# rayglover-ibm/sparse-solvers

Measured on AMD Instinct MI355X. Metric: signals recovered/sec (Homotopy l1, m=8192 n=65536 k=64 fp32), higher is better.
Workload: dtype f32; 1 GPU; configs[1]: one signal per solve, A 8192x65536 fp32 = default_rng(1234).standard_normal/sqrt(m) (SURVEY 8d recipe), k=64 positive coefficients, tol 1e-3, max_iter 256; shipped defaults (reference behaviour: tie_guard 0, zero_on_removal 0); m=8192, n=65536, k=64, sweep_variant=5, engine=1

## Files before the change

### sparse-solvers_amd/csrc/resident.hip

```cpp
#include "ss_hip_internal.h"
#include "ss_hip_device.h"
#include "resident.h"

#include <hip/hip_fp16.h>

#include <algorithm>
#include <cmath>
#include <cstdio>
#include <cstdlib>
#include <cstring>

namespace sship {

template <typename T> struct ResVec;
template <> struct ResVec<double> { typedef double v2 __attribute__((ext_vector_type(2))); };
template <> struct ResVec<float>  { typedef float v2 __attribute__((ext_vector_type(2))); };

template <typename T>
struct ResLds {
    T* I;
    T* dvec;
    T* xvec;
    T* u1sg;
    T* u2w;
    int32_t* posof;
    uint32_t* subc;
    uint32_t* pcol;
    uint32_t* psub;
};

template <typename T>
__host__ __device__ inline size_t res_lds_bytes()
{
    typedef ResCfg<T> C;
    return ((size_t)C::PCAP * (C::PCAP + 1) + 6 * (size_t)C::PCAP) * sizeof(T) + ((size_t)2 * C::S + 2 * (size_t)C::PCAP) * 4;
}

template <typename T> __device__ __forceinline__ T res_sqrt(T v);
template <> __device__ __forceinline__ float res_sqrt<float>(float v) { return sqrtf(v); }
template <> __device__ __forceinline__ double res_sqrt<double>(double v) { return sqrt(v); }
template <typename T> __device__ __forceinline__ T res_fma(T a, T b, T c);
template <> __device__ __forceinline__ float res_fma<float>(float a, float b, float c) { return __builtin_fmaf(a, b, c); }
template <> __device__ __forceinline__ double res_fma<double>(double a, double b, double c) { return __builtin_fma(a, b, c); }
template <typename T> __device__ __forceinline__ T res_abs(T v) { return v < T(0) ? -v : v; }

__device__ __forceinline__ uint32_t uni(uint32_t v) { return (uint32_t)__builtin_amdgcn_readfirstlane((int)v); }
__device__ __forceinline__ int32_t uni(int32_t v) { return __builtin_amdgcn_readfirstlane(v); }
__device__ __forceinline__ float uni(float v) { return __uint_as_float(uni(__float_as_uint(v))); }
__device__ __forceinline__ double uni(double v)
{
    const uint32_t lo = uni((uint32_t)__double2loint(v)), hi = uni((uint32_t)__double2hiint(v));
    return __hiloint2double((int)hi, (int)lo);
}


__device__ __forceinline__ void cmov_inplace(float& dst, float src, unsigned long long msk)
{
    asm volatile("v_cndmask_b32_e64 %0, %0, %1, %2" : "+v"(dst) : "v"(src), "s"(msk));
}
__device__ __forceinline__ void cmov_inplace(double& dst, double src, unsigned long long msk)
{
    uint32_t lo = (uint32_t)__double2loint(dst), hi = (uint32_t)__double2hiint(dst);
    const uint32_t slo = (uint32_t)__double2loint(src), shi = (uint32_t)__double2hiint(src);
    asm volatile("v_cndmask_b32_e64 %0, %0, %2, %4\n\tv_cndmask_b32_e64 %1, %1, %3, %4" : "+v"(lo), "+v"(hi) : "v"(slo), "v"(shi), "s"(msk));
    dst = __hiloint2double((int)hi, (int)lo);
}

template <typename T>
__device__ __forceinline__ T group8_sum(T v)
{
    v += dpp_mov<kDppXor1>(v);
    v += dpp_mov<kDppXor2>(v);
    v += dpp_mov<kDppHalfMirror>(v);
    return v;
}

template <typename T>
__device__ __forceinline__ T wave_max_val(T v)
{
    { const T o = dpp_mov<kDppXor1>(v); v = o > v ? o : v; }
    { const T o = dpp_mov<kDppXor2>(v); v = o > v ? o : v; }
    { const T o = dpp_mov<kDppHalfMirror>(v); v = o > v ? o : v; }
    { const T o = dpp_mov<kDppMirror>(v); v = o > v ? o : v; }
    T b = lane_value(v, 0);
#pragma unroll
    for (int r = 1; r < 4; ++r) { const T o = lane_value(v, 16 * r); b = o > b ? o : b; }
    return b;
}

constexpr uint32_t kPickNone = 0xffffu;
template <typename T> struct alignas(16) ResPick { T v; uint32_t who; uint32_t col; };
static_assert(sizeof(ResPick<float>) == 16 && sizeof(ResPick<double>) == 16, "one 16-byte read per wave");

template <typename T, bool OMP, bool STAMPS = false>
__global__ __launch_bounds__(ResCfg<T>::THREADS)
void k_res_solve(const T* __restrict__ Gs_all, uint32_t gpitch, size_t g_slot_stride, const T* __restrict__ c0_all, uint32_t c0_stride,
                 const uint32_t* __restrict__ sub_all, uint32_t n, T tol, uint32_t max_iter, int strict_sign, int tie_guard, int tie_exit,
                 uint32_t kcap, uint32_t* __restrict__ log_hdr, T* __restrict__ log_H, uint32_t* __restrict__ log_pcol, T* __restrict__ log_X, T* __restrict__ log_D,
                 T* __restrict__ x_all, uint32_t x_stride, uint32_t* __restrict__ gam2_all, uint32_t* __restrict__ touched2_all,
                 DevState* __restrict__ st_all, TraceEntry* trace, uint32_t trace_cap, unsigned long long* dbg = nullptr)
{
    unsigned long long tph[6] = { 0, 0, 0, 0, 0, 0 };
    unsigned long long tlast = 0;
#define RES_STAMP(PH) if constexpr (STAMPS) { const unsigned long long now_ = __builtin_readcyclecounter(); tph[PH] += now_ - tlast; tlast = now_; }
    typedef ResCfg<T> C;
    typedef typename ResVec<T>::v2 V2;
    constexpr uint32_t S = C::S, THREADS = C::THREADS, PCAP = C::PCAP, LOGCAP = C::LOGCAP;
    constexpr int CT = C::CT, PT = C::PCAP / 8;
    constexpr uint32_t NW = (THREADS + 63) / 64;
    constexpr uint32_t IP = PCAP + 1u;
    static_assert(THREADS / 8 * CT == S, "eight lanes per column group");
    static_assert(PCAP % 8 == 0 && (CT == 4 || CT == 8), "positions dealt out over the eight lanes of a group");
    extern __shared__ __attribute__((aligned(16))) unsigned char smem[];
    __shared__ T s_max[16];
    __shared__ ResPick<T> s_pick[NW];
    __shared__ T s_f[4];
    ResLds<T> L;
    {
        T* p = reinterpret_cast<T*>(smem);
        L.I = p; p += (size_t)PCAP * IP;
        L.dvec = p; p += PCAP; L.xvec = p; p += PCAP; L.u1sg = p; p += 2 * PCAP; L.u2w = p; p += 2 * PCAP;
        L.posof = reinterpret_cast<int32_t*>(p);
        L.subc = reinterpret_cast<uint32_t*>(L.posof + S);
        L.pcol = L.subc + S;
        L.psub = L.pcol + PCAP;
    }
    const uint32_t slot = blockIdx.x, t = threadIdx.x, lane = t & 63u, wave = t >> 6;
    const uint32_t grp = t >> 3, g = t & 7u;
    const T* Gs = Gs_all + (size_t)slot * g_slot_stride;
    const T* c0 = c0_all + (size_t)slot * c0_stride;
    const uint32_t* sub = sub_all + (size_t)slot * S;
    T* x_out = x_all + (size_t)slot * x_stride;
    uint32_t* gam_out = gam2_all + (size_t)slot * 2 * kcap;
    uint32_t* tch_out = touched2_all + (size_t)slot * 2 * kcap;
    DevState* st = st_all + slot;
    uint32_t* hdr = log_hdr + (size_t)slot * LOGCAP * 8;
    T* LH = log_H != nullptr ? log_H + (size_t)slot * LOGCAP * 2 : nullptr;
    T* LX = log_X + (size_t)slot * LOGCAP * PCAP;
    T* LD = log_D != nullptr ? log_D + (size_t)slot * LOGCAP * PCAP : nullptr;
    if (slot != 0) trace = nullptr;

    const uint32_t jc0 = grp * (uint32_t)CT;
    const bool owner = g < (uint32_t)CT;
    const uint32_t myj = jc0 + (g & (uint32_t)(CT - 1));
    const uint32_t mycol = sub[myj];
    const bool myvalid = owner && mycol < n;
    const T my_c0 = mycol < n ? c0[mycol] : T(0);
    T my_c = my_c0, my_q = T(0);
    int32_t mypos = -1;
    T gr[CT][PT];
#pragma unroll
    for (int c = 0; c < CT; ++c)
#pragma unroll
        for (int e = 0; e < PT; ++e) gr[c][e] = T(0);
    for (uint32_t j = t; j < S; j += THREADS) { L.subc[j] = sub[j]; L.posof[j] = -1; }
    for (uint32_t p = t; p < PCAP; p += THREADS) {
        L.dvec[p] = T(0); L.xvec[p] = T(0); L.pcol[p] = 0xffffffffu; L.psub[p] = 0u;
        L.u1sg[2 * p] = T(0); L.u1sg[2 * p + 1] = T(0); L.u2w[2 * p] = T(0); L.u2w[2 * p + 1] = T(0);
    }
    for (uint32_t e = t; e < PCAP * IP; e += THREADS) L.I[e] = T(0);
    T warm = T(0);
    {
        const size_t gbytes = (size_t)S * gpitch * sizeof(T);
        const unsigned char* gb = reinterpret_cast<const unsigned char*>(Gs);
#pragma unroll 4
        for (size_t off = (size_t)t * 128u; off < gbytes; off += (size_t)THREADS * 128u) warm += *reinterpret_cast<const T*>(gb + off);
    }

    auto publish_pick = [&](T v, T ext, bool tiew) __attribute__((always_inline)) {
        const unsigned long long bal = __builtin_amdgcn_ballot_w64(v == ext);
        const uint32_t src = bal != 0ull ? (uint32_t)__builtin_ctzll(bal) : 0u;
        if (lane == src) {
            ResPick<T> sl;
            sl.v = ext;
            sl.who = (myvalid ? myj : kPickNone) | ((uint32_t)(mypos + 1) << 16) | (tiew ? 0x80000000u : 0u);
            sl.col = mycol;
            s_pick[wave] = sl;
        }
    };
    auto gather_pick = [&](bool want_min, T& v, uint32_t& i, uint32_t& col, int32_t& pos, bool& tie) __attribute__((always_inline)) {
        ResPick<T> sl[NW];
#pragma unroll
        for (uint32_t w = 0; w < NW; ++w) sl[w] = s_pick[w];
        T bv = sl[0].v;
        uint32_t bw = sl[0].who, bc = sl[0].col, ties = sl[0].who;
#pragma unroll
        for (uint32_t w = 1; w < NW; ++w) {
            const bool take = want_min ? sl[w].v < bv : sl[w].v > bv;
            bv = take ? sl[w].v : bv; bw = take ? sl[w].who : bw; bc = take ? sl[w].col : bc;
            ties |= sl[w].who;
        }
        v = uni(bv);
        const uint32_t who = uni((bw & 0x7fffffffu) | (ties & 0x80000000u));
        col = uni(bc);
        i = (who & 0xffffu) == kPickNone ? 0xffffffffu : (who & 0xffffu);
        pos = (int32_t)((who >> 16) & 0x7fffu) - 1;
        tie = (who >> 31) != 0u;
    };
    auto block_min = [&](T m, bool tie, T& v, uint32_t& i, uint32_t& col, int32_t& pos, bool& anytie) __attribute__((always_inline)) {
        publish_pick(m, -wave_max_val<T>(-m), __builtin_amdgcn_ballot_w64(tie) != 0ull);
        lds_barrier();
        gather_pick(true, v, i, col, pos, anytie);
    };
    auto block_argmax = [&](T m, T& v, uint32_t& i, uint32_t& col, int32_t& pos) __attribute__((always_inline)) {
        const T wv = wave_max_val<T>(m);
        lds_barrier();
        publish_pick(m, wv, false);
        lds_barrier();
        bool none;
        gather_pick(false, v, i, col, pos, none);
        lds_barrier();
    };
    auto border_inverse = [&](uint32_t P, T dvv) __attribute__((always_inline)) {
        constexpr uint32_t RW = PCAP / 2u + 1u;
        constexpr uint32_t NG = THREADS / RW;
        const uint32_t Pn = P + 1u;
        const uint32_t pa = t % RW, vg = t / RW;
        const uint32_t a0 = pa, a1 = Pn - 1u - pa;
        if (P != 0xffffffffu && vg < NG && 2u * pa < Pn + 1u - 0u && a0 <= a1) {
            const uint32_t n0 = Pn - a0;
            const uint32_t ntot = a0 == a1 ? n0 : n0 + (Pn - a1);
            const T u0 = a0 < P ? L.u2w[2 * a0] : T(0), u1v = a1 < P ? L.u2w[2 * a1] : T(0);
            constexpr uint32_t BU = sizeof(T) == 8 ? 2u : 3u;
            auto where = [&](uint32_t k, uint32_t& a, uint32_t& b, T& ua) __attribute__((always_inline)) {
                const bool first = k < n0;
                a = first ? a0 : a1;
                b = first ? a0 + k : a1 + (k - n0);
                ua = first ? u0 : u1v;
            };
            auto value = [&](uint32_t a, uint32_t b, T ua, T iv, T ub) __attribute__((always_inline)) -> T {
                const T edge = a == P ? dvv : -dvv * ua;
                const T inner = iv + (dvv * ua) * ub;
                return b == P ? edge : inner;
            };
            uint32_t k = vg;
#pragma nounroll
            for (; k + (BU - 1u) * NG < ntot; k += BU * NG) {
                uint32_t ea[BU], eb[BU];
                T ua[BU], iv[BU], ub[BU];
#pragma unroll
                for (uint32_t u = 0; u < BU; ++u) {
                    where(k + u * NG, ea[u], eb[u], ua[u]);
                    iv[u] = L.I[ea[u] * IP + eb[u]];
                    ub[u] = L.u2w[2 * eb[u]];
                }
#pragma unroll
                for (uint32_t u = 0; u < BU; ++u) {
                    const T val = value(ea[u], eb[u], ua[u], iv[u], ub[u]);
                    L.I[ea[u] * IP + eb[u]] = val;
                    L.I[eb[u] * IP + ea[u]] = val;
                }
            }
#pragma nounroll
            for (; k < ntot; k += NG) {
                uint32_t ea, eb;
                T ua;
                where(k, ea, eb, ua);
                const T val = value(ea, eb, ua, L.I[ea * IP + eb], L.u2w[2 * eb]);
                L.I[ea * IP + eb] = val;
                L.I[eb * IP + ea] = val;
            }
        }
    };

    struct RowVals { T mine; T gv[CT]; };
    auto row_fetch = [&](uint32_t spi, RowVals& rv) __attribute__((always_inline)) {
        const T* row = Gs + (size_t)spi * gpitch;
        rv.mine = row[myj];
        if constexpr (sizeof(T) == 8) {
            const v2d a = *reinterpret_cast<const v2d*>(row + jc0), b = *reinterpret_cast<const v2d*>(row + jc0 + 2);
            rv.gv[0] = a[0]; rv.gv[1] = a[1]; rv.gv[2] = b[0]; rv.gv[3] = b[1];
        } else {
            const v4f a = *reinterpret_cast<const v4f*>(row + jc0), b = *reinterpret_cast<const v4f*>(row + jc0 + 4);
#pragma unroll
            for (int e = 0; e < 4; ++e) { rv.gv[e] = a[e]; rv.gv[4 + e] = b[e]; }
        }
        asm volatile("" ::: "memory");
    };
    auto row_place = [&](uint32_t Pn, const RowVals& rv) __attribute__((always_inline)) {
        const uint32_t e_new = uni(Pn >> 3);
        const unsigned long long msk = __builtin_amdgcn_ballot_w64(g == (Pn & 7u));
#pragma unroll
        for (int c = 0; c < CT; ++c) asm volatile("" :: "v"(rv.gv[c]));
        asm volatile("" :: "v"(rv.mine));
        if constexpr (CT == 8) {
#define RES_CM(I) "v_cndmask_b32_e64 %[d" #I "], %[d" #I "], %[s" #I "], %[m]\n\t"
#pragma unroll
            for (int e = 0; e < PT; ++e) {
                const uint32_t off = uni(e_new ^ (uint32_t)e);
                asm volatile("s_cmp_lg_u32 %[off], 0\n\t"
                             "s_cbranch_scc1 .Lres_place_%=\n\t"
                             RES_CM(0) RES_CM(1) RES_CM(2) RES_CM(3) RES_CM(4) RES_CM(5) RES_CM(6) RES_CM(7)
                             ".Lres_place_%=:"
                             : [d0] "+v"(gr[0][e]), [d1] "+v"(gr[1][e]), [d2] "+v"(gr[2][e]), [d3] "+v"(gr[3][e]), [d4] "+v"(gr[4][e]), [d5] "+v"(gr[5][e]),
                               [d6] "+v"(gr[6][e]), [d7] "+v"(gr[7][e])
                             : [s0] "v"(rv.gv[0]), [s1] "v"(rv.gv[1]), [s2] "v"(rv.gv[2]), [s3] "v"(rv.gv[3]), [s4] "v"(rv.gv[4]), [s5] "v"(rv.gv[5]),
                               [s6] "v"(rv.gv[6]), [s7] "v"(rv.gv[7]), [m] "s"(msk), [off] "s"(off)
                             : "scc");
            }
#undef RES_CM
        } else {
#pragma unroll
            for (int e = 0; e < PT; ++e) {
                if (e_new == (uint32_t)e) {
#pragma unroll
                    for (int c = 0; c < CT; ++c) cmov_inplace(gr[c][e], rv.gv[c], msk);
                }
            }
        }
    };
    auto chain = [&](const T* vec, uint32_t P) __attribute__((always_inline)) -> T {
        T acc[CT];
#pragma unroll
        for (int c = 0; c < CT; ++c) acc[c] = T(0);
#pragma unroll
        for (int e = 0; e < PT; ++e) {
            if ((uint32_t)(8 * e) < P) {
                const T dval = vec[8 * e + (int)g];
#pragma unroll
                for (int c = 0; c < CT; ++c) acc[c] = res_fma<T>(dval, gr[c][e], acc[c]);
            }
        }
        T h4[4];
        if constexpr (CT == 8) {
            const bool up = (g & 4u) != 0u;
#pragma unroll
            for (int i = 0; i < 4; ++i) {
                const T keep = up ? acc[4 + i] : acc[i], send = up ? acc[i] : acc[4 + i];
                h4[i] = keep + dpp_mov<kDppHalfMirror>(send);
            }
        } else {
#pragma unroll
            for (int i = 0; i < 4; ++i) h4[i] = acc[i] + dpp_mov<kDppHalfMirror>(acc[i]);
        }
        const bool b1 = (g & 2u) != 0u, b0 = (g & 1u) != 0u;
        const T k0 = (b1 ? h4[2] : h4[0]) + dpp_mov<kDppXor2>(b1 ? h4[0] : h4[2]);
        const T k1 = (b1 ? h4[3] : h4[1]) + dpp_mov<kDppXor2>(b1 ? h4[1] : h4[3]);
        return (b0 ? k1 : k0) + dpp_mov<kDppXor1>(b0 ? k0 : k1);
    };
    auto inverse_pass = [&](uint32_t P) __attribute__((always_inline)) {
        constexpr int CH = sizeof(T) == 8 ? 6 : PT;
        for (uint32_t a = grp; a < P; a += THREADS / 8u) {
            const T* row = L.I + (size_t)a * IP + g;
            const T* us = L.u1sg + 2u * g;
            T s1 = T(0), s2 = T(0);
#pragma nounroll
            for (int e0 = 0; e0 < PT; e0 += CH) {
                if ((uint32_t)(8 * e0) < P) {
                    T iv[CH];
                    V2 pr[CH];
#pragma unroll
                    for (int e = 0; e < CH; ++e) {
                        if (e0 + e < PT) {
                            iv[e] = row[8 * (e0 + e)];
                            pr[e] = *reinterpret_cast<const V2*>(&us[16 * (e0 + e)]);
                        } else { iv[e] = T(0); pr[e] = V2{ T(0), T(0) }; }
                    }
#pragma unroll
                    for (int e = 0; e < CH; ++e) {
                        s1 = res_fma<T>(iv[e], pr[e][0], s1);
                        s2 = res_fma<T>(iv[e], pr[e][1], s2);
                    }
                }
            }
            s1 = group8_sum<T>(s1); s2 = group8_sum<T>(s2);
            if (g == 0) { L.u2w[2 * a] = s1; L.u2w[2 * a + 1] = s2; }
        }
    };
    auto two_dots = [&](uint32_t P, T& d1, T& d2) __attribute__((always_inline)) {
        T a1 = T(0), a2 = T(0);
#pragma nounroll
        for (uint32_t b = lane; b < P; b += 64u) {
            const V2 pr = *reinterpret_cast<const V2*>(&L.u1sg[2 * b]);
            const T u2b = L.u2w[2 * b];
            a1 = res_fma<T>(pr[0], u2b, a1);
            a2 = res_fma<T>(u2b, pr[1], a2);
        }
        d1 = wave_sum<T>(a1); d2 = wave_sum<T>(a2);
    };
    asm volatile("" : "+s"(trace_cap));
    uint32_t P = 0, status = 0, iter = 0, nlog = 0, reason = 0;
    T c_inf = T(0), lambda_prev = T(0), gamma_prev = T(0), lambda0 = T(0);
    bool tie_any = false;
    lds_barrier();

    uint32_t sp0;
    {
        uint32_t col0;
        int32_t pos0;
        block_argmax(myvalid ? res_abs<T>(my_c) : T(-1), lambda0, sp0, col0, pos0);
    }
    if (sp0 >= S) { status = kStatusSubsetDecline; reason |= kReasonNoCand; }
    else {
        RowVals rv0;
        row_fetch(sp0, rv0);
        row_place(0u, rv0);
        const T g00 = rv0.mine;
        if (owner && myj == sp0) {
            const T nrm = res_sqrt<T>(g00);
            const T inv00 = T(1) / (nrm * nrm);
            const T seed = strict_sign ? my_c : res_abs<T>(my_c);
            const T sg0 = sign_tol<T>(seed, tol);
            L.I[0] = inv00;
            if (OMP) L.xvec[0] = inv00 * my_c; else L.dvec[0] = inv00 * sg0;
            L.pcol[0] = mycol; L.psub[0] = sp0; L.posof[sp0] = 0;
            mypos = 0;
            if (!OMP && trace != nullptr) { trace[0].idx = mycol; trace[0].added = 1; trace[0].gamma = 0.0; trace[0].c_inf = (double)res_abs<T>(my_c); }
        }
        P = 1;
        c_inf = lambda0;
        lambda_prev = lambda0;
        if (!((double)tol >= (sizeof(T) == 8 ? kGramGuard64 : kGramGuard) * (double)lambda0)) { status = kStatusSubsetDecline; reason |= kReasonGuard; }
        lds_barrier();
    }

    if constexpr (OMP) {
        if (status == 0u && !(lambda0 > tol)) { status = kStatusSubsetDecline; reason |= kReasonNoCand; }
        if (status == 0u) {
            if (t == 0) {
                uint32_t* h = hdr;
                h[0] = 0u; h[1] = 1u; h[2] = L.subc[sp0]; h[3] = 1u; h[4] = __float_as_uint((float)lambda0); h[5] = 0u; h[6] = 0xffffffffu; h[7] = 0u;
                if (LH != nullptr) { LH[0] = lambda0; LH[1] = T(0); }
                if (trace != nullptr && 1u < trace_cap) { trace[1].idx = L.subc[sp0]; trace[1].added = 1u; trace[1].gamma = 0.0; trace[1].c_inf = (double)lambda0; }
            }
            if (t < PCAP) LX[t] = T(0);
            nlog = 1;
            iter = 1;
        }
        for (uint32_t round = 2; status == 0u; ++round) {
            my_c = my_c0 - chain(L.xvec, P);
            uint32_t bi, idx;
            int32_t wpos;
            block_argmax(myvalid ? res_abs<T>(my_c) : T(-1), c_inf, bi, idx, wpos);
            const uint32_t spi = bi < S ? bi : 0u;
            RowVals rv;
            row_fetch(spi, rv);
            const bool stop = !(c_inf > tol) || round > max_iter;
            const bool logfull = nlog >= LOGCAP;
            const bool stall_c = bi >= S || wpos >= 0;
            const bool full_c = P >= PCAP || P + 1u > kcap;
            uint32_t verdict = full_c ? kReasonPositions : 0u;
            verdict = stall_c ? (uint32_t)kReasonNoCand : verdict;
            verdict = stop ? 0u : verdict;
            verdict = logfull ? (uint32_t)kReasonLog : verdict;
            const bool ok = !stop && verdict == 0u;
            const bool ends = stop && !logfull;
            status = verdict != 0u ? (uint32_t)kStatusSubsetDecline : ends ? 0xffffffffu : status;
            reason |= verdict;
            iter = ends ? round - 1 : iter;
            row_place(ok ? P : 0xffffffffu, rv);
            const T my_g = rv.mine;
            if (owner && mypos >= 0) { L.u1sg[2 * mypos] = my_g; L.u1sg[2 * mypos + 1] = my_c0; }
            if (ok && owner && myj == spi) { s_f[0] = my_g; s_f[1] = my_c0; L.posof[spi] = (int32_t)P; L.pcol[P] = idx; L.psub[P] = spi; mypos = (int32_t)P; }
            lds_barrier();
            if (!logfull) {
                if (t == 0) {
                    uint32_t* h = hdr + nlog * 8;
                    h[0] = P; h[1] = stop ? 0u : 1u; h[2] = ok ? idx : 0xffffffffu; h[3] = ok ? 1u : 0u; h[4] = __float_as_uint((float)c_inf); h[5] = 0u;
                    h[6] = 0xffffffffu; h[7] = 0u;
                    if (LH != nullptr) { LH[nlog * 2] = c_inf; LH[nlog * 2 + 1] = T(0); }
                    if (ok && trace != nullptr && round < trace_cap) { trace[round].idx = idx; trace[round].added = 1u; trace[round].gamma = 0.0; trace[round].c_inf = (double)c_inf; }
                }
                if (t < PCAP) LX[(size_t)nlog * PCAP + t] = t < P ? L.xvec[t] : T(0);
                ++nlog;
            }
            inverse_pass(P);
            lds_barrier();
            T d1, d2;
            two_dots(P, d1, d2);
            const T dvv = T(1) / (s_f[0] - d1);
            const T beta = dvv * (s_f[1] - d2);
            if (ok && t < P) L.xvec[t] = L.u2w[2 * t + 1] - beta * L.u2w[2 * t];
            if (ok && t == P) L.xvec[P] = beta;
            border_inverse(ok ? P : 0xffffffffu, dvv);
            lds_barrier();
            if (ok) { P += 1u; iter = round; }
        }
        if (status == 0xffffffffu) status = 0u;
    } else {
        if (status == 0u) my_q = chain(L.dvec, P);
        uint32_t pendP = 0xffffffffu;
        T pend_dv = T(0);
        constexpr uint32_t TL0 = THREADS - ((PCAP + 63u) / 64u) * 64u;
        const uint32_t tl = t - TL0;
        for (uint32_t round = 1; status == 0u; ++round) {
            if constexpr (STAMPS) tlast = __builtin_readcyclecounter();
            const bool stop = (round > 1 && !(c_inf > tol)) || round > max_iter;
            const bool logfull = nlog >= LOGCAP;
            const bool in_band = tie_band<T>(c_inf, lambda_prev, gamma_prev, lambda0);
            T m = Lim<T>::max();
            bool tie = false;
            if (myvalid) {
                if (mypos >= 0) {
                    const T tt = -L.xvec[mypos] / L.dvec[mypos];
                    if (tt > T(0) && tt < m) m = tt;
                } else {
                    const T dl = T(1) - my_q, dr = T(1) + my_q;
                    if (dl != T(0)) {
                        T tt = (c_inf - my_c) / dl;
                        if (tie_guard && tt == T(0) && dl > T(0)) tt = Lim<T>::tiny();
                        if (tt == T(0) && in_band) tie = true;
                        if (tt > T(0) && tt < m) m = tt;
                    }
                    if (dr != T(0)) {
                        T tt = (c_inf + my_c) / dr;
                        if (tie_guard && tt == T(0) && dr > T(0)) tt = Lim<T>::tiny();
                        if (tt == T(0) && in_band) tie = true;
                        if (tt > T(0) && tt < m) m = tt;
                    }
                }
            }
            T gmm;
            uint32_t bi, idx;
            int32_t wpos;
            bool anytie;
            block_min(m, tie, gmm, bi, idx, wpos, anytie);
            RES_STAMP(0)
            const uint32_t spi = bi < S ? bi : 0u;
            RowVals rv;
            row_fetch(spi, rv);
            tie_any = tie_any || (!stop && anytie);
            const bool tied_c = tie_any && tie_exit != 0;
            const bool nocand_c = bi >= S || !(gmm < Lim<T>::max());
            const bool full_c = P >= PCAP || P + 1u > kcap;
            uint32_t verdict = full_c ? kReasonPositions : 0u;
            verdict = wpos >= 0 ? (uint32_t)kReasonRemoval : verdict;
            verdict = nocand_c ? (uint32_t)kReasonNoCand : verdict;
            verdict = tied_c ? (uint32_t)kReasonTie : verdict;
            verdict = stop ? 0u : verdict;
            verdict = logfull ? (uint32_t)kReasonLog : verdict;
            const bool ok = !stop && verdict == 0u;
            const bool ends = stop && !logfull;
            const bool tied = verdict == kReasonTie;
            status = ends ? 0xffffffffu : tied ? (uint32_t)kStatusTieRerun : verdict != 0u ? (uint32_t)kStatusSubsetDecline : status;
            reason |= verdict;
            iter = ends || tied ? round - 1 : iter;
            T xv = T(0), dv = T(0);
            if (tl < P) { xv = L.xvec[tl]; dv = L.dvec[tl]; }
            border_inverse(pendP, pend_dv);
            pendP = 0xffffffffu;
            if (ok && tl < P) L.xvec[tl] = xv + gmm * dv;
            if (ok) my_c = res_fma<T>(-gmm, my_q, my_c);
            {
                const T mx = wave_max_val<T>(myvalid ? res_abs<T>(my_c) : T(-1));
                if (lane == 0) s_max[wave] = mx;
            }
            row_place(ok ? P : 0xffffffffu, rv);
            const T my_g = rv.mine;
            if (owner && mypos >= 0) { L.u1sg[2 * mypos] = my_g; L.u1sg[2 * mypos + 1] = sign_tol<T>(my_c, tol); }
            if (ok && owner && myj == spi) {
                s_f[0] = my_g; s_f[1] = sign_tol<T>(my_c, tol);
                L.posof[spi] = (int32_t)P; L.pcol[P] = idx; L.psub[P] = spi; mypos = (int32_t)P;
            }
            lds_barrier();
            RES_STAMP(1)
            if (!logfull) {
                if (tl == 0u) {
                    uint32_t* h = hdr + nlog * 8;
                    h[0] = P; h[1] = stop ? 0u : 1u; h[2] = ok ? idx : 0xffffffffu; h[3] = ok ? 1u : 0u; h[4] = __float_as_uint((float)c_inf);
                    h[5] = ok ? __float_as_uint((float)gmm) : 0u; h[6] = 0xffffffffu; h[7] = in_band ? 1u : 0u;
                    if (LH != nullptr) { LH[nlog * 2] = c_inf; LH[nlog * 2 + 1] = ok ? gmm : T(0); }
                    if (ok && trace != nullptr && round < trace_cap) { trace[round].idx = idx; trace[round].added = 1u; trace[round].gamma = (double)gmm; trace[round].c_inf = (double)c_inf; }
                }
                if (tl < PCAP) {
                    LX[(size_t)nlog * PCAP + tl] = xv;
                    if (LD != nullptr) LD[(size_t)nlog * PCAP + tl] = dv;
                }
                if (stop || tied || ok) ++nlog;
            }
            T c_next = s_max[0];
#pragma unroll
            for (uint32_t w = 1; w < NW; ++w) { const T o = s_max[w]; c_next = o > c_next ? o : c_next; }
            c_next = uni(c_next);
            inverse_pass(P);
            lds_barrier();
            RES_STAMP(2)
            T d1, d2;
            two_dots(P, d1, d2);
            const T dvv = T(1) / (s_f[0] - d1);
            const T beta = dvv * (s_f[1] - d2);
            if (ok && t < P) L.dvec[t] = L.u2w[2 * t + 1] - beta * L.u2w[2 * t];
            if (ok && t == P) L.dvec[P] = beta;
            pendP = ok ? P : 0xffffffffu;
            pend_dv = dvv;
            lds_barrier();
            RES_STAMP(3)
            if (ok) {
                P += 1u;
                lambda_prev = c_inf;
                gamma_prev = gmm;
                c_inf = c_next;
                iter = round;
            }
            my_q = chain(L.dvec, P);
            RES_STAMP(4)
            if constexpr (STAMPS) tph[5] += 1;
        }
        if (status == 0xffffffffu) status = 0u;
    }
    if constexpr (STAMPS) {
        if (dbg != nullptr && slot == 0u && t == 0u)
            for (int q = 0; q < 6; ++q) dbg[q] = tph[q];
    }
#undef RES_STAMP
    lds_barrier();
    if (t < PCAP) log_pcol[(size_t)slot * PCAP + t] = t < P ? L.pcol[t] : 0xffffffffu;
    if (status == 0u || status == kStatusTieRerun) {
        if (t < P) {
            const uint32_t col = L.pcol[t];
            uint32_t rk = 0;
#pragma nounroll
            for (uint32_t b = 0; b < P; ++b) rk += L.pcol[b] < col ? 1u : 0u;
            gam_out[rk] = col;
            tch_out[rk] = col;
            x_out[col] = L.xvec[t];
        }
    }
    if (t == 0) {
        st->done = 1;
        st->status = status;
        st->iter = iter;
        st->K = P;
        st->ntouched = P;
        st->cur = 0;
        st->c_inf = (double)c_inf;
        st->gamma = (double)gamma_prev;
        st->tie_stall = tie_any ? 1u : 0u;
        st->lambda0 = (float)lambda0;
        st->solo_nlog = nlog;
        st->need_sweep = 0;
        st->done_round = iter + 1u;
        st->sub_reason = reason;
    }
    if (warm == T(1.2345e-30)) st->pad4_[0] = 1u;
}

constexpr uint32_t kG64T = 64, kG64Step = 32, kG64Pitch = kG64Step + 1;
typedef double res_v4d __attribute__((ext_vector_type(4)));

__global__ __launch_bounds__(256)
void k_sgram64_part(const double* __restrict__ At, uint32_t ldm, uint32_t n, const uint32_t* __restrict__ sub, uint32_t rows_per,
                    double* __restrict__ part)
{
    constexpr uint32_t S = ResCfg<double>::S;
    __shared__ double sI[kG64T][kG64Pitch];
    __shared__ double sJ[kG64T][kG64Pitch];
    sub += (size_t)blockIdx.z * S;
    part += (size_t)blockIdx.z * gridDim.y * S * S;
    const uint32_t b = blockIdx.x;
    uint32_t tt = (uint32_t)((__fsqrt_rn(8.f * (float)b + 1.f) - 1.f) * 0.5f);
    while (tt * (tt + 1u) / 2u > b) --tt;
    while ((tt + 1u) * (tt + 2u) / 2u <= b) ++tt;
    const uint32_t bj = tt, bi = b - tt * (tt + 1u) / 2u;
    const uint32_t chunk = blockIdx.y;
    const uint32_t tid = threadIdx.x, lane = tid & 63u, w = tid >> 6;
    const uint32_t wi = w >> 1, wj = w & 1u;
    const uint32_t sc = tid >> 2, sq = tid & 3u;
    const uint32_t ci = sub[bi * kG64T + sc], cj = sub[bj * kG64T + sc];
    const bool oki = ci < n, okj = cj < n;
    const double* gi = At + (size_t)(oki ? ci : 0u) * ldm + (size_t)chunk * rows_per + 8u * sq;
    const double* gj = At + (size_t)(okj ? cj : 0u) * ldm + (size_t)chunk * rows_per + 8u * sq;
    const v2d zero2 = { 0.0, 0.0 };
    v2d vi[4], vj[4];
#define SG64_LOAD(R0)                                                                         \
    _Pragma("unroll") for (int p = 0; p < 4; ++p) {                                           \
        vi[p] = oki ? *reinterpret_cast<const v2d*>(gi + (R0) + 2 * p) : zero2;               \
        vj[p] = okj ? *reinterpret_cast<const v2d*>(gj + (R0) + 2 * p) : zero2;               \
    }
    SG64_LOAD(0u)
    res_v4d acc[2][2];
#pragma unroll
    for (int i = 0; i < 2; ++i)
#pragma unroll
        for (int j = 0; j < 2; ++j) acc[i][j] = res_v4d{ 0.0, 0.0, 0.0, 0.0 };
    const uint32_t l15 = lane & 15u, kq = lane >> 4;
    for (uint32_t r0 = 0; r0 < rows_per; r0 += kG64Step) {
        __syncthreads();
#pragma unroll
        for (int p = 0; p < 4; ++p) {
            sI[sc][8u * sq + 2u * (uint32_t)p] = vi[p][0]; sI[sc][8u * sq + 2u * (uint32_t)p + 1u] = vi[p][1];
            sJ[sc][8u * sq + 2u * (uint32_t)p] = vj[p][0]; sJ[sc][8u * sq + 2u * (uint32_t)p + 1u] = vj[p][1];
        }
        __syncthreads();
        if (r0 + kG64Step < rows_per) SG64_LOAD(r0 + kG64Step)
#pragma unroll
        for (uint32_t k4 = 0; k4 < kG64Step; k4 += 4) {
            const double a0 = sI[32u * wi + l15][k4 + kq], a1 = sI[32u * wi + 16u + l15][k4 + kq];
            const double b0 = sJ[32u * wj + l15][k4 + kq], b1 = sJ[32u * wj + 16u + l15][k4 + kq];
            acc[0][0] = __builtin_amdgcn_mfma_f64_16x16x4f64(a0, b0, acc[0][0], 0, 0, 0);
            acc[0][1] = __builtin_amdgcn_mfma_f64_16x16x4f64(a0, b1, acc[0][1], 0, 0, 0);
            acc[1][0] = __builtin_amdgcn_mfma_f64_16x16x4f64(a1, b0, acc[1][0], 0, 0, 0);
            acc[1][1] = __builtin_amdgcn_mfma_f64_16x16x4f64(a1, b1, acc[1][1], 0, 0, 0);
        }
    }
#undef SG64_LOAD
    double* Pp = part + (size_t)chunk * S * S;
#pragma unroll
    for (int i = 0; i < 2; ++i)
#pragma unroll
        for (int j = 0; j < 2; ++j)
#pragma unroll
            for (int e = 0; e < 4; ++e) {
                const uint32_t row = bi * kG64T + 32u * wi + 16u * (uint32_t)i + 4u * (uint32_t)e + kq;
                const uint32_t col = bj * kG64T + 32u * wj + 16u * (uint32_t)j + l15;
                Pp[(size_t)row * S + col] = acc[i][j][e];
                if (bi != bj) Pp[(size_t)col * S + row] = acc[i][j][e];
            }
}

__global__ __launch_bounds__(256)
void k_sgram64_sum(const double* __restrict__ part, uint32_t nsplit, double* __restrict__ gs, const double* __restrict__ At, uint32_t ldm,
                   const double* __restrict__ y, const uint32_t* __restrict__ sub, uint32_t n, double* __restrict__ c0, uint32_t c0_stride)
{
    constexpr uint32_t S = ResCfg<double>::S;
    constexpr uint32_t NB = S * S / 256u;
    {
        const size_t slot = blockIdx.y;
        part += slot * nsplit * S * S; gs += slot * S * S; y += slot * ldm; sub += slot * S; c0 += slot * c0_stride;
    }
    if (blockIdx.x >= NB) {
        __shared__ double sv[16];
        const uint32_t col = sub[blockIdx.x - NB];
        const double* a = At + (size_t)(col < n ? col : 0u) * ldm;
        double acc = 0.0;
        for (uint32_t r0 = 2u * threadIdx.x; r0 < ldm; r0 += 8u * 512u) {
            v2d av[8], yv[8];
#pragma unroll
            for (int q = 0; q < 8; ++q) {
                const uint32_t r = r0 + 512u * (uint32_t)q;
                av[q] = r < ldm ? *reinterpret_cast<const v2d*>(a + r) : v2d{ 0.0, 0.0 };
                yv[q] = r < ldm ? *reinterpret_cast<const v2d*>(y + r) : v2d{ 0.0, 0.0 };
            }
#pragma unroll
            for (int q = 0; q < 8; ++q) { acc = __builtin_fma(av[q][0], yv[q][0], acc); acc = __builtin_fma(av[q][1], yv[q][1], acc); }
        }
        acc = block_sum(acc, sv);
        if (threadIdx.x == 0u && col < n) c0[col] = acc;
        return;
    }
    const uint32_t i = blockIdx.x * 256u + threadIdx.x;
    double s = part[i];
    for (uint32_t c = 1; c < nsplit; ++c) s += part[(size_t)c * S * S + i];
    gs[i] = s;
}

constexpr uint32_t kR64Rhs = 192;
__device__ __forceinline__ float res_state_scale(float lam_eff)
{
    int e = 12;
    if (lam_eff > 0.f && lam_eff < 3.0e38f) e = (int)floorf(log2f(4096.f / lam_eff));
    e = e < -100 ? -100 : (e > 100 ? 100 : e);
    return ldexpf(1.f, e);
}

__global__ __launch_bounds__(256)
void k_res_residuals64(const double* __restrict__ At, uint32_t ldm, uint32_t n, const double* __restrict__ y, const uint32_t* __restrict__ hdr,
                       const double* __restrict__ LH, const uint32_t* __restrict__ pcol, const double* __restrict__ LX, double tol,
                       const float* __restrict__ meta, __half* __restrict__ r16, float* __restrict__ rn2p, float* __restrict__ tab,
                       uint32_t* __restrict__ headroom, DevState* __restrict__ st, int first16, int omp, const float* __restrict__ slotmeta,
                       uint32_t* __restrict__ fl, int scan)
{
    constexpr uint32_t kFlCap = kScrFlCap;
    constexpr uint32_t PCAP = ResCfg<double>::PCAP;
    constexpr uint32_t LOGCAP = ResCfg<double>::LOGCAP;
    constexpr uint32_t XP = kR64Rhs + 8u;
    {
        const size_t slot = blockIdx.y;
        y += slot * ldm; hdr += slot * LOGCAP * 8; LH += slot * LOGCAP * 2; pcol += slot * PCAP; LX += slot * LOGCAP * PCAP;
        r16 += slot * kR64Rhs * ldm; rn2p += slot * (ldm / 64u) * kR64Rhs; tab += slot * kR64Rhs * 4u; st += slot;
        if (slotmeta != nullptr) slotmeta += slot * 4u;
    }
    __shared__ __attribute__((aligned(16))) double sAc[16][64];
    __shared__ __attribute__((aligned(16))) double sXt[16][XP];
    __shared__ float sS[kR64Rhs];
    if (st->status != 0u && !scan) return;
    const uint32_t tid = threadIdx.x, r0 = blockIdx.x * 64u;
    const uint32_t nlog = st->solo_nlog;
    float ratio0 = 0.f;
    if (fl != nullptr && blockIdx.x == 0u && blockIdx.y == 0u && tid == 0u) {
        fl[0] = 0u; fl[kFlCap + 1u] = 0u; fl[kFlCap + 4u] = 0u; fl[kFlCap + 12u] = 0u; fl[kFlCap + 13u] = 0u;
        if (!scan) fl[kFlCap + 14u] = 0u;
    }
    if (first16 && !scan && blockIdx.x == 0u && tid == 0u && nlog >= 1u) {
        const float lam0 = (float)LH[0] * 0.9999999f;
        const float yn = sqrtf(slotmeta != nullptr ? slotmeta[0] : meta[5]) * 1.001f;
        float eps0 = slotmeta != nullptr ? 0.0019726562f * yn * meta[4] + 6.103515625e-05f * sqrtf((float)ldm) * yn * meta[1]
                                         : meta[8] * yn * meta[4] + meta[9] * sqrtf((float)ldm) * yn;
        if (slotmeta != nullptr) eps0 += 6.103515625e-05f * sqrtf((float)ldm) * meta[4] * slotmeta[2];
        const float bound0 = lam0 * 0.875f - 1e-12f * lam0;
        const float v0 = (slotmeta != nullptr ? slotmeta[1] : meta[6]) + eps0;
        if (!(v0 <= bound0)) {
            if (fl != nullptr && bound0 > 0.f) { fl[kFlCap + 1u] = 1u; fl[kFlCap + 2u] = __float_as_uint(bound0); fl[kFlCap + 3u] = __float_as_uint(eps0); }
            else { __hip_atomic_store(&st->need_sweep, 1u, __ATOMIC_RELAXED, __HIP_MEMORY_SCOPE_AGENT); atomicOr(&st->sub_reason, kReasonFirstState); }
        }
        ratio0 = bound0 > 0.f && v0 == v0 ? v0 / bound0 : 3.0e38f;
    }
    if (nlog < 2u) {
        if (blockIdx.x == 0u && tid == 0u && blockIdx.y == 0u) *headroom = __float_as_uint(ratio0);
        return;
    }
    const uint32_t nst = nlog - 1u;
    if (nst > kR64Rhs) {
        if (blockIdx.x == 0u && tid == 0u && !scan) { __hip_atomic_store(&st->need_sweep, 1u, __ATOMIC_RELAXED, __HIP_MEMORY_SCOPE_AGENT); atomicOr(&st->sub_reason, kReasonLog); }
        return;
    }
    const uint32_t Pfin = hdr[(size_t)(nlog - 1u) * 8u];
    if (tid < kR64Rhs) {
        float sc = 1.f;
        if (tid < nst) {
            const double lam = LH[(size_t)(tid + 1u) * 2u];
            const bool final_state = !(hdr[(size_t)(tid + 1u) * 8u + 1u] & 1u);
            sc = res_state_scale((float)(final_state ? fmax(lam, tol) : lam));
        }
        sS[tid] = sc;
    }
    const uint32_t rg = tid & 15u, sgp = tid >> 4;
    double acc[3][4][4];
    {
        const v2d y0 = *reinterpret_cast<const v2d*>(y + r0 + 4u * rg), y1 = *reinterpret_cast<const v2d*>(y + r0 + 4u * rg + 2u);
#pragma unroll
        for (int rd = 0; rd < 3; ++rd)
#pragma unroll
            for (int si = 0; si < 4; ++si) { acc[rd][si][0] = y0[0]; acc[rd][si][1] = y0[1]; acc[rd][si][2] = y1[0]; acc[rd][si][3] = y1[1]; }
    }
    for (uint32_t u0 = 0; u0 < Pfin; u0 += 16u) {
        __syncthreads();
        {
            const uint32_t p = tid >> 4, q4 = tid & 15u;
            const uint32_t u = u0 + p;
            const uint32_t col = u < Pfin ? pcol[u] : 0xffffffffu;
            v2d a0 = { 0.0, 0.0 }, a1 = { 0.0, 0.0 };
            if (col < n) {
                a0 = *reinterpret_cast<const v2d*>(At + (size_t)col * ldm + r0 + 4u * q4);
                a1 = *reinterpret_cast<const v2d*>(At + (size_t)col * ldm + r0 + 4u * q4 + 2u);
            }
            *reinterpret_cast<v2d*>(&sAc[p][4u * q4]) = a0;
            *reinterpret_cast<v2d*>(&sAc[p][4u * q4 + 2u]) = a1;
            for (uint32_t e = tid; e < 16u * XP; e += 256u) {
                const uint32_t k = e / 16u, pp = e - k * 16u;
                sXt[pp][k] = (u0 + pp < Pfin && k < nst) ? LX[(size_t)(k + 1u) * PCAP + u0 + pp] : 0.0;
            }
        }
        __syncthreads();
#pragma unroll
        for (int rd = 0; rd < 3; ++rd) {
            const uint32_t s0 = 64u * (uint32_t)rd + 4u * sgp;
            if (s0 < nst) {
#pragma unroll 4
                for (uint32_t p = 0; p < 16u; ++p) {
                    const v2d a0 = *reinterpret_cast<const v2d*>(&sAc[p][4u * rg]), a1 = *reinterpret_cast<const v2d*>(&sAc[p][4u * rg + 2u]);
                    const v2d x0 = *reinterpret_cast<const v2d*>(&sXt[p][s0]), x1 = *reinterpret_cast<const v2d*>(&sXt[p][s0 + 2u]);
                    const double av[4] = { a0[0], a0[1], a1[0], a1[1] }, xv[4] = { x0[0], x0[1], x1[0], x1[1] };
#pragma unroll
                    for (int si = 0; si < 4; ++si)
#pragma unroll
                        for (int ri = 0; ri < 4; ++ri) acc[rd][si][ri] = __builtin_fma(-xv[si], av[ri], acc[rd][si][ri]);
                }
            }
        }
    }
    const double units = (double)meta[13];
    bool ovf = false;
#pragma unroll
    for (int rd = 0; rd < 3; ++rd) {
#pragma unroll
        for (int si = 0; si < 4; ++si) {
            const uint32_t kk = 64u * (uint32_t)rd + 4u * sgp + (uint32_t)si;
            const float sc = sS[kk < kR64Rhs ? kk : 0u];
            float ss = 0.f;
            __half hv[4];
#pragma unroll
            for (int ri = 0; ri < 4; ++ri) {
                const float r = (float)(acc[rd][si][ri] * units);
                ss = __builtin_fmaf(r, r, ss);
                const float v = r * sc;
                if (kk < nst && !(fabsf(v) < 60000.f)) ovf = true;
                hv[ri] = __float2half_rn(v);
            }
            ss += __shfl_xor(ss, 1); ss += __shfl_xor(ss, 2); ss += __shfl_xor(ss, 4); ss += __shfl_xor(ss, 8);
            if (kk < nst) {
                *reinterpret_cast<uint2*>(r16 + (size_t)kk * ldm + r0 + 4u * rg) = *reinterpret_cast<const uint2*>(hv);
                if (rg == 0u) rn2p[(size_t)blockIdx.x * kR64Rhs + kk] = ss * 1.0001f;
            }
        }
    }
    if (ovf && !scan) { __hip_atomic_store(&st->need_sweep, 1u, __ATOMIC_RELAXED, __HIP_MEMORY_SCOPE_AGENT); atomicOr(&st->sub_reason, kReasonOverflow); }
    if (blockIdx.x == 0u) {
        if (tid == 0u && blockIdx.y == 0u) *headroom = __float_as_uint(ratio0);
        if (tid < nst) {
            const uint32_t* hh = hdr + (size_t)(tid + 1u) * 8u;
            const uint32_t* hp = hdr + (size_t)tid * 8u;
            const double lam_d = LH[(size_t)(tid + 1u) * 2u];
            const double lam_pd = LH[(size_t)tid * 2u], gam_pd = LH[(size_t)tid * 2u + 1u];
            const float lam = (float)lam_d;
            const bool final_state = !(hh[1] & 1u);
            const float slack = 1e-12f * (float)LH[0];
            float bound;
            if (omp) {
                bound = (final_state && !(lam_d > tol) ? (float)tol * 0.9375f : lam * 0.875f) - slack;
            } else {
                const double lam_exp = lam_pd - gam_pd;
                const bool ls_jump = final_state && !(lam_d > tol) && !(lam_exp > 1e-13 * LH[0]);
                if (ls_jump) bound = (float)tol * 0.9375f - slack;
                else bound = fminf(lam, (float)lam_exp) * 0.875f - slack;
                const bool irregular = hp[3] == 0u || lam_d > lam_pd * (1.0 + 1e-12);
                if (irregular && !scan) {
                    bound = -1.f;
                    atomicOr(&st->sub_reason, kReasonIrregular);
                    __hip_atomic_store(&st->need_sweep, 1u, __ATOMIC_RELAXED, __HIP_MEMORY_SCOPE_AGENT);
                }
                if (scan && (irregular || final_state)) bound = 3.0e38f;
            }
            const float inv_sk = 1.f / sS[tid];
            tab[tid * 4u + 0] = (meta[1] * meta[12]) * inv_sk;
            tab[tid * 4u + 1] = bound;
            tab[tid * 4u + 2] = inv_sk;
            tab[tid * 4u + 3] = lam;
        }
    }
}

template <typename T>
bool res_solve_usable()
{
    static const bool ok = [] {
        const hipError_t e = hipFuncSetAttribute(reinterpret_cast<const void*>(&k_res_solve<T, false>), hipFuncAttributeMaxDynamicSharedMemorySize,
                                                 (int)res_lds_bytes<T>());
        const hipError_t e2 = hipFuncSetAttribute(reinterpret_cast<const void*>(&k_res_solve<T, true>), hipFuncAttributeMaxDynamicSharedMemorySize,
                                                  (int)res_lds_bytes<T>());
        if (e != hipSuccess || e2 != hipSuccess) (void)hipGetLastError();
        return e == hipSuccess && e2 == hipSuccess;
    }();
    return ok;
}
template bool res_solve_usable<float>();
template bool res_solve_usable<double>();

template <typename T>
hipError_t launch_res_solve(ss_hip_ctx* ctx, uint32_t nslots, const T* Gs, uint32_t gpitch, size_t g_slot_stride, const T* c0, uint32_t c0_stride,
                            const uint32_t* sub, T tol, uint32_t max_iter, uint32_t kcap, const ResLog<T>& log, T* x, uint32_t x_stride,
                            uint32_t* gam2, uint32_t* touched2, DevState* st, TraceEntry* trace, uint32_t trace_cap, bool omp)
{
    if (!res_solve_usable<T>()) return hipErrorInvalidConfiguration;
    static unsigned long long* dbg = nullptr;
    static const bool stamps = std::getenv("SS_HIP_RES_STAMPS") != nullptr;
    if (stamps && !omp) {
        static const bool ok = [] {
            const bool a = hipFuncSetAttribute(reinterpret_cast<const void*>(&k_res_solve<T, false, true>), hipFuncAttributeMaxDynamicSharedMemorySize,
                                               (int)res_lds_bytes<T>()) == hipSuccess;
            return a && hipMalloc(&dbg, 8 * sizeof(unsigned long long)) == hipSuccess;
        }();
        if (ok) {
            hipLaunchKernelGGL((k_res_solve<T, false, true>), dim3(nslots), dim3(ResCfg<T>::THREADS), res_lds_bytes<T>(), ctx->stream, Gs, gpitch, g_slot_stride, c0, c0_stride,
                               sub, (uint32_t)ctx->n, tol, max_iter, ctx->strict_sign, ctx->tie_guard, (ctx->tie_rerun && !ctx->tie_guard) ? 1 : 0, kcap,
                               log.hdr, log.H, log.pcol, log.X, log.D, x, x_stride, gam2, touched2, st, trace, trace_cap, dbg);
            unsigned long long tp[6];
            if (hipMemcpyAsync(tp, dbg, sizeof(tp), hipMemcpyDeviceToHost, ctx->stream) == hipSuccess && hipStreamSynchronize(ctx->stream) == hipSuccess) {
                const double r = tp[5] ? (double)tp[5] : 1.0;
                std::fprintf(stderr, "[k_res_solve<%s>, cycles per round over %llu rounds] scan+argmin %.0f  row+border+x+c %.0f  log+inverse pass %.0f  dots+dir %.0f  chain %.0f\n",
                             sizeof(T) == 8 ? "double" : "float", tp[5], tp[0] / r, tp[1] / r, tp[2] / r, tp[3] / r, tp[4] / r);
            }
            return hipGetLastError();
        }
    }
    if (omp)
        hipLaunchKernelGGL((k_res_solve<T, true>), dim3(nslots), dim3(ResCfg<T>::THREADS), res_lds_bytes<T>(), ctx->stream, Gs, gpitch, g_slot_stride, c0, c0_stride,
                           sub, (uint32_t)ctx->n, tol, max_iter, ctx->strict_sign, ctx->tie_guard, (ctx->tie_rerun && !ctx->tie_guard) ? 1 : 0, kcap,
                           log.hdr, log.H, log.pcol, log.X, log.D, x, x_stride, gam2, touched2, st, trace, trace_cap);
    else
        hipLaunchKernelGGL((k_res_solve<T, false>), dim3(nslots), dim3(ResCfg<T>::THREADS), res_lds_bytes<T>(), ctx->stream, Gs, gpitch, g_slot_stride, c0, c0_stride,
                           sub, (uint32_t)ctx->n, tol, max_iter, ctx->strict_sign, ctx->tie_guard, (ctx->tie_rerun && !ctx->tie_guard) ? 1 : 0, kcap,
                           log.hdr, log.H, log.pcol, log.X, log.D, x, x_stride, gam2, touched2, st, trace, trace_cap);
    return hipGetLastError();
}
template hipError_t launch_res_solve<float>(ss_hip_ctx*, uint32_t, const float*, uint32_t, size_t, const float*, uint32_t, const uint32_t*, float, uint32_t,
                                            uint32_t, const ResLog<float>&, float*, uint32_t, uint32_t*, uint32_t*, DevState*, TraceEntry*, uint32_t, bool);
template hipError_t launch_res_solve<double>(ss_hip_ctx*, uint32_t, const double*, uint32_t, size_t, const double*, uint32_t, const uint32_t*, double, uint32_t,
                                             uint32_t, const ResLog<double>&, double*, uint32_t, uint32_t*, uint32_t*, DevState*, TraceEntry*, uint32_t, bool);

hipError_t launch_sgram64(ss_hip_ctx* ctx, const uint32_t* sub, const double* y, double* part, double* gs, double* c0, uint32_t nslots, uint32_t c0_stride)
{
    constexpr uint32_t S = ResCfg<double>::S, NT = S / kG64T;
    const uint32_t ldm = ctx->ldm;
    uint32_t nsplit = ldm / 512u;
    if (nsplit == 0u || ldm % (nsplit * kG64Step) != 0u) nsplit = ldm / 256u;
    if (nsplit > kSg64MaxSplit) nsplit = kSg64MaxSplit;
    while (nsplit > 1u && ldm % (nsplit * kG64Step) != 0u) --nsplit;
    const double* At = static_cast<const double*>(ctx->At);
    hipLaunchKernelGGL(k_sgram64_part, dim3(NT * (NT + 1) / 2, nsplit, nslots), dim3(256), 0, ctx->stream, At, ldm, (uint32_t)ctx->n, sub, ldm / nsplit, part);
    hipLaunchKernelGGL(k_sgram64_sum, dim3(S * S / 256u + S, nslots), dim3(256), 0, ctx->stream, (const double*)part, nsplit, gs, At, ldm, y, sub, (uint32_t)ctx->n, c0,
                       c0_stride);
    return hipGetLastError();
}

hipError_t launch_res_residuals64(ss_hip_ctx* ctx, const double* y, const ResLog<double>& log, double tol, const float* meta, void* r16, float* rn2p,
                                  float* tab, uint32_t* headroom, DevState* st, bool first16, bool omp, uint32_t nslots, const float* slotmeta, uint32_t* fl, bool scan)
{
    hipLaunchKernelGGL(k_res_residuals64, dim3(ctx->ldm / 64u, nslots), dim3(256), 0, ctx->stream, static_cast<const double*>(ctx->At), ctx->ldm, (uint32_t)ctx->n, y,
                       (const uint32_t*)log.hdr, (const double*)log.H, (const uint32_t*)log.pcol, (const double*)log.X, tol, meta,
                       static_cast<__half*>(r16), rn2p, tab, headroom, st, first16 ? 1 : 0, omp ? 1 : 0, slotmeta, fl, scan ? 1 : 0);
    return hipGetLastError();
}

}
```

Measured before the change: 1778 signals/s.

## Fuse border inverse update into inverse pass and hoist stop test out of loop

For fp32, the rank-one border update of the inverse Gram matrix is folded into the next inverse_pass. Each row element is updated and used for the u2 dot products in the same sweep, which saves a separate read-modify-write pass over the inverse and its barrier. The update operands are stored in a new LDS array u2p, which enlarges shared memory. The stop condition is also moved into the loop header, and the final log entry is written after the loop, so the last round no longer runs a full iteration just to stop. The log and status handling on exit is reimplemented, which risks small behavioural differences.

```diff
diff --git a/sparse-solvers_amd/csrc/resident.hip b/sparse-solvers_amd/csrc/resident.hip
--- a/sparse-solvers_amd/csrc/resident.hip
+++ b/sparse-solvers_amd/csrc/resident.hip
@@ -23,6 +23,7 @@
     T* xvec;
     T* u1sg;
     T* u2w;
+    T* u2p;
     int32_t* posof;
     uint32_t* subc;
     uint32_t* pcol;
@@ -33,7 +34,7 @@
 __host__ __device__ inline size_t res_lds_bytes()
 {
     typedef ResCfg<T> C;
-    return ((size_t)C::PCAP * (C::PCAP + 1) + 6 * (size_t)C::PCAP) * sizeof(T) + ((size_t)2 * C::S + 2 * (size_t)C::PCAP) * 4;
+    return ((size_t)C::PCAP * (C::PCAP + 1) + 8 * (size_t)C::PCAP) * sizeof(T) + ((size_t)2 * C::S + 2 * (size_t)C::PCAP) * 4;
 }
 
 template <typename T> __device__ __forceinline__ T res_sqrt(T v);
@@ -119,7 +120,7 @@
     {
         T* p = reinterpret_cast<T*>(smem);
         L.I = p; p += (size_t)PCAP * IP;
-        L.dvec = p; p += PCAP; L.xvec = p; p += PCAP; L.u1sg = p; p += 2 * PCAP; L.u2w = p; p += 2 * PCAP;
+        L.dvec = p; p += PCAP; L.xvec = p; p += PCAP; L.u1sg = p; p += 2 * PCAP; L.u2w = p; p += 2 * PCAP; L.u2p = p; p += 2 * PCAP;
         L.posof = reinterpret_cast<int32_t*>(p);
         L.subc = reinterpret_cast<uint32_t*>(L.posof + S);
         L.pcol = L.subc + S;
@@ -156,7 +157,7 @@
     for (uint32_t j = t; j < S; j += THREADS) { L.subc[j] = sub[j]; L.posof[j] = -1; }
     for (uint32_t p = t; p < PCAP; p += THREADS) {
         L.dvec[p] = T(0); L.xvec[p] = T(0); L.pcol[p] = 0xffffffffu; L.psub[p] = 0u;
-        L.u1sg[2 * p] = T(0); L.u1sg[2 * p + 1] = T(0); L.u2w[2 * p] = T(0); L.u2w[2 * p + 1] = T(0);
+        L.u1sg[2 * p] = T(0); L.u1sg[2 * p + 1] = T(0); L.u2w[2 * p] = T(0); L.u2w[2 * p + 1] = T(0); L.u2p[2 * p] = T(0); L.u2p[2 * p + 1] = T(0);
     }
     for (uint32_t e = t; e < PCAP * IP; e += THREADS) L.I[e] = T(0);
     T warm = T(0);
@@ -367,6 +368,37 @@
             if (g == 0) { L.u2w[2 * a] = s1; L.u2w[2 * a + 1] = s2; }
         }
     };
+    auto inverse_pass_fused = [&](uint32_t P, uint32_t pendP) __attribute__((always_inline)) {
+        for (uint32_t a = grp; a < P; a += THREADS / 8u) {
+            T* row = L.I + (size_t)a * IP + g;
+            const T* us = L.u1sg + 2u * g;
+            const T* up = L.u2p + 2u * g;
+            const V2 ta = *reinterpret_cast<const V2*>(&L.u2p[2 * a]);
+            const V2 pa = V2{ ta[1], ta[0] };
+            const int32_t diag = (int32_t)a - (int32_t)g;
+            T s1 = T(0), s2 = T(0);
+            T iv[PT];
+            V2 pr[PT], pb[PT];
+#pragma unroll
+            for (int e = 0; e < PT; ++e) {
+                iv[e] = row[8 * e];
+                pr[e] = *reinterpret_cast<const V2*>(&us[16 * e]);
+                pb[e] = *reinterpret_cast<const V2*>(&up[16 * e]);
+            }
+#pragma unroll
+            for (int e = 0; e < PT; ++e) {
+                if ((uint32_t)(8 * e) <= pendP) {
+                    const V2 prod = pa * pb[e];
+                    iv[e] = iv[e] + (diag <= 8 * e ? prod[1] : prod[0]);
+                    row[8 * e] = iv[e];
+                }
+                s1 = res_fma<T>(iv[e], pr[e][0], s1);
+                s2 = res_fma<T>(iv[e], pr[e][1], s2);
+            }
+            s1 = group8_sum<T>(s1); s2 = group8_sum<T>(s2);
+            if (g == 0) { L.u2w[2 * a] = s1; L.u2w[2 * a + 1] = s2; }
+        }
+    };
     auto two_dots = [&](uint32_t P, T& d1, T& d2) __attribute__((always_inline)) {
         T a1 = T(0), a2 = T(0);
 #pragma nounroll
@@ -479,13 +511,17 @@
         if (status == 0xffffffffu) status = 0u;
     } else {
         if (status == 0u) my_q = chain(L.dvec, P);
+        constexpr bool FUSED = sizeof(T) == 4;
         uint32_t pendP = 0xffffffffu;
         T pend_dv = T(0);
         constexpr uint32_t TL0 = THREADS - ((PCAP + 63u) / 64u) * 64u;
         const uint32_t tl = t - TL0;
-        for (uint32_t round = 1; status == 0u; ++round) {
+        constexpr bool SHORT = sizeof(T) == 4;
+        uint32_t round = 1;
+        auto stop_at = [&](uint32_t r) __attribute__((always_inline)) { return (r > 1 && !(c_inf > tol)) || r > max_iter; };
+        for (; status == 0u && !(SHORT && stop_at(round)); ++round) {
             if constexpr (STAMPS) tlast = __builtin_readcyclecounter();
-            const bool stop = (round > 1 && !(c_inf > tol)) || round > max_iter;
+            const bool stop = !SHORT && stop_at(round);
             const bool logfull = nlog >= LOGCAP;
             const bool in_band = tie_band<T>(c_inf, lambda_prev, gamma_prev, lambda0);
             T m = Lim<T>::max();
@@ -537,8 +573,7 @@
             iter = ends || tied ? round - 1 : iter;
             T xv = T(0), dv = T(0);
             if (tl < P) { xv = L.xvec[tl]; dv = L.dvec[tl]; }
-            border_inverse(pendP, pend_dv);
-            pendP = 0xffffffffu;
+            if constexpr (!FUSED) border_inverse(pendP, pend_dv);
             if (ok && tl < P) L.xvec[tl] = xv + gmm * dv;
             if (ok) my_c = res_fma<T>(-gmm, my_q, my_c);
             {
@@ -572,15 +607,22 @@
 #pragma unroll
             for (uint32_t w = 1; w < NW; ++w) { const T o = s_max[w]; c_next = o > c_next ? o : c_next; }
             c_next = uni(c_next);
-            inverse_pass(P);
+            if (FUSED && pendP != 0xffffffffu) inverse_pass_fused(P, pendP); else inverse_pass(P);
             lds_barrier();
             RES_STAMP(2)
             T d1, d2;
             two_dots(P, d1, d2);
             const T dvv = T(1) / (s_f[0] - d1);
             const T beta = dvv * (s_f[1] - d2);
-            if (ok && t < P) L.dvec[t] = L.u2w[2 * t + 1] - beta * L.u2w[2 * t];
-            if (ok && t == P) L.dvec[P] = beta;
+            if (ok && t < P) {
+                const T u2t = L.u2w[2 * t];
+                L.dvec[t] = L.u2w[2 * t + 1] - beta * u2t;
+                if constexpr (FUSED) *reinterpret_cast<V2*>(&L.u2p[2 * t]) = V2{ dvv * u2t, u2t };
+            }
+            if (ok && t == P) {
+                L.dvec[P] = beta;
+                if constexpr (FUSED) *reinterpret_cast<V2*>(&L.u2p[2 * P]) = V2{ -dvv, T(-1) };
+            }
             pendP = ok ? P : 0xffffffffu;
             pend_dv = dvv;
             lds_barrier();
@@ -597,6 +639,22 @@
             if constexpr (STAMPS) tph[5] += 1;
         }
         if (status == 0xffffffffu) status = 0u;
+        else if (SHORT && status == 0u) {
+            if (nlog < LOGCAP) {
+                if (tl == 0u) {
+                    uint32_t* h = hdr + nlog * 8;
+                    h[0] = P; h[1] = 0u; h[2] = 0xffffffffu; h[3] = 0u; h[4] = __float_as_uint((float)c_inf);
+                    h[5] = 0u; h[6] = 0xffffffffu; h[7] = tie_band<T>(c_inf, lambda_prev, gamma_prev, lambda0) ? 1u : 0u;
+                    if (LH != nullptr) { LH[nlog * 2] = c_inf; LH[nlog * 2 + 1] = T(0); }
+                }
+                if (tl < PCAP) {
+                    LX[(size_t)nlog * PCAP + tl] = tl < P ? L.xvec[tl] : T(0);
+                    if (LD != nullptr) LD[(size_t)nlog * PCAP + tl] = tl < P ? L.dvec[tl] : T(0);
+                }
+                ++nlog;
+                iter = round - 1;
+            } else { status = kStatusSubsetDecline; reason |= kReasonLog; }
+        }
     }
     if constexpr (STAMPS) {
         if (dbg != nullptr && slot == 0u && t == 0u)
```

Result: no change. 1794 signals/s, median of 6 (+0.9%).
